# M4THYOU/TokenDagger

Measured on AMD Instinct MI355X. Metric: GB/s raw text tokenized (Llama-4 vocab, 1024 MB corpus), higher is better.
Workload: dtype u8; 1 GPU; Llama-4-Scout vocab, 1024 MiB synthetic english text, 1741775 documents, CoreBPE::encode semantics, input resident in HBM; bytes=1073741824, docs=1741775, bytes_rank0=1073741824, docs_rank0=1741775, parallelism=single GPU

## Files before the change

tokendagger_amd/csrc/td_kernels.hip:

```cpp
#include <hip/hip_runtime.h>
#include <stdlib.h>

#include "td_kernels.h"

namespace td {

#ifdef TD_ABLATE
#define TD_STOP(n) (a.stop_after == (n))
#else
#define TD_STOP(n) false
#endif

struct LdsSrc {
    const uint8_t* txt;
    const uint32_t* docw;
    int64_t lo, hi;
    __device__ __forceinline__ uint32_t byte(int64_t i) const { return txt[i]; }
    __device__ __forceinline__ bool doc(int64_t i) const { return (docw[i >> 5] >> (i & 31)) & 1u; }
};
struct GlobSrc {
    const uint8_t* text;
    const uint32_t* docbits;
    int64_t lo, hi;
    __device__ __forceinline__ uint32_t byte(int64_t i) const { return text[i]; }
// ... 3858 lines not shown
        bool fast_this = false;
        uint4 sx0 = cx0, sx1 = cx0, sx2 = cx0, sx3 = cx0;
        uint32_t sh0 = 0, stl = 0, sdsl = 0;
        int64_t sdpos = 0;
        if (SKIP_PLAIN && lane_walk) {
            bool done = false;
            while (!lw_cur) {
                if (!lw_nz) {
                    lw_base += nwaves * 64;
                    if (lw_base >= n_mwords) { done = true; break; }
                    lw_mine = lw_base + lane < n_mwords ? (walk_all ? 0xFFFFu : (uint32_t)a.rest_mask[lw_base + lane]) : 0u;
                    lw_nz = __ballot(lw_mine != 0u);
                    if (!lw_nz) continue;
                }
                const int l = td_ctz64(lw_nz);
                lw_nz &= lw_nz - 1ull;
                lw_cur = (uint32_t)__shfl((int)lw_mine, l);
                lw_index = lw_base + l;
            }
            if (done) break;
            const int bq = (int)td_ctz32(lw_cur);
            lw_cur &= lw_cur - 1u;
            tile = lw_index * 16 + bq;
            if (tile >= a.n_tiles) continue;
            tc = a.tile_count[tile]; ex = a.tile_extra[tile]; dfirst = (int64_t)a.tile_first_doc[tile];
            base = a.tile_base[tile] + a.chunk_pref[tile / K_SCAN_CHUNK];
            if (pk_simple(tc, base, ex, a.out_cap) || (a.pack_dense && pk_dense(tc, base, ex, a.out_cap))) continue;
        } else if constexpr (SKIP_PLAIN) {
            if (!cmask) {
                t0 += 4 * nwaves;
                if (t0 >= a.n_tiles) break;
                uint32_t w[4] = {0, 0, 0, 0};
#pragma unroll
                for (int q = 0; q < 4; ++q) {
                    const int tq = t0 + q * nwaves;
                    if (tq < a.n_tiles) w[q] = walk_all ? 0xFFFFu : (uint32_t)a.rest_mask[tq >> 4];
                }
#pragma unroll
                for (int q = 0; q < 4; ++q) {
                    const int tq = t0 + q * nwaves;
                    if (tq < a.n_tiles && ((w[q] >> (tq & 15)) & 1u)) cmask |= 1u << q;
                }
#pragma unroll
                for (int q = 0; q < 4; ++q) {
                    const int tq = t0 + q * nwaves;
                    if ((cmask >> q) & 1u) {
                        c_tc[q] = a.tile_count[tq]; c_ex[q] = a.tile_extra[tq]; c_df[q] = a.tile_first_doc[tq];
                        c_base[q] = a.tile_base[tq] + a.chunk_pref[tq / K_SCAN_CHUNK];
                    }
                }
                if (!cmask) continue;
            }
            const int q = (int)td_ctz32(cmask);
            cmask &= cmask - 1u;
            tile = t0 + q * nwaves;
            tc = q == 0 ? c_tc[0] : q == 1 ? c_tc[1] : q == 2 ? c_tc[2] : c_tc[3];
            ex = q == 0 ? c_ex[0] : q == 1 ? c_ex[1] : q == 2 ? c_ex[2] : c_ex[3];
            dfirst = (int64_t)(q == 0 ? c_df[0] : q == 1 ? c_df[1] : q == 2 ? c_df[2] : c_df[3]);
            base = q == 0 ? c_base[0] : q == 1 ? c_base[1] : q == 2 ? c_base[2] : c_base[3];
            if (pk_simple(tc, base, ex, a.out_cap) || (a.pack_dense && pk_dense(tc, base, ex, a.out_cap))) continue;
        } else {
            tile += nwaves;
            if (tile >= a.n_tiles) break;
            if (tile + 2 * nwaves < a.n_tiles) PK_FETCH(tile + 2 * nwaves, C)
            const bool fast_next = tile + nwaves < a.n_tiles && PK_FAST(B);
            if (fast_next) PK_LOAD(tile + nwaves, B, n)
            tc = tcA;
            base = baseA;
            dfirst = (int64_t)dfA;
            fast_this = fast_cur;
            sx0 = cx0; sx1 = cx1; sx2 = cx2; sx3 = cx3;
            sh0 = ch0; stl = ctl; sdsl = cdsl;
            sdpos = cdpos;
            tcA = tcB; baseA = baseB; dfA = dfB; tcB = tcC; baseB = baseC; dfB = dfC;
            fast_cur = fast_next;
            cx0 = nx0; cx1 = nx1; cx2 = nx2; cx3 = nx3; ch0 = nh0; ctl = ntl; cdsl = ndsl; cdpos = ndpos;
        }
        (void)ex;
        if (PLAIN_ONLY && !fast_this) continue;
        if (tc & TILE_DIRECT) {
            if (tile == a.n_tiles - 1) {
                const int64_t d_end = lower_bound_i64(a.doc_offsets, a.n_docs, a.n);
                for (int64_t d = d_end + lane; d <= a.n_docs; d += 64) a.out_offsets[d] = total;
            }
            continue;
        }
        if (fast_this && !TD_STOP(61)) {
            const uint32_t g_c = tc & TILE_COUNT_MASK;
            int32_t* dst = a.out_tokens + base;
            uint32_t g_head = (uint32_t)((16u - ((uint32_t)(uintptr_t)dst & 15u)) & 15u) >> 2;
            if (g_head > g_c) g_head = g_c;
            const uint32_t g_nv = (g_c - g_head) >> 2, g_done = g_head + 4 * g_nv;
            if ((uint32_t)lane < g_nv) *reinterpret_cast<uint4*>(dst + g_head + 4 * lane) = sx0;
            if ((uint32_t)lane + 64 < g_nv) *reinterpret_cast<uint4*>(dst + g_head + 4 * (lane + 64)) = sx1;
            if ((uint32_t)lane + 128 < g_nv) *reinterpret_cast<uint4*>(dst + g_head + 4 * (lane + 128)) = sx2;
            if ((uint32_t)lane + 192 < g_nv) *reinterpret_cast<uint4*>(dst + g_head + 4 * (lane + 192)) = sx3;
            if ((uint32_t)lane < g_head) dst[lane] = (int32_t)sh0;
            if (g_done + (uint32_t)lane < g_c) dst[g_done + lane] = (int32_t)stl;
            const int64_t g_lo = (int64_t)tile * K_TILE;
            const int64_t g_hi = (g_lo + K_TILE < a.n) ? g_lo + K_TILE : a.n;
            const int64_t dm = dfirst + lane;
            if (sdpos < g_hi) a.out_offsets[dm] = base + sdsl;
            if (__all(sdpos < g_hi)) {
                for (int64_t d = dfirst + 64 + lane; d < a.n_docs; d += 64) {
                    if (a.doc_offsets[d] >= g_hi) break;
                    a.out_offsets[d] = base + a.doc_slot[d];
                }
            }
            if (tile == a.n_tiles - 1) {
                const int64_t d_end = lower_bound_i64(a.doc_offsets, a.n_docs, a.n);
                for (int64_t d = d_end + lane; d <= a.n_docs; d += 64) a.out_offsets[d] = total;
            }
            continue;
        }
        if constexpr (PLAIN_ONLY) continue;
        const uint32_t cnt = tc & TILE_COUNT_MASK;
        const uint32_t* src = a.stage + (size_t)tile * K_STAGE;
        const int64_t g_lo = (int64_t)tile * K_TILE;
        const int64_t g_hi = (g_lo + K_TILE < a.n) ? g_lo + K_TILE : a.n;
        PK_TICK(t_meta)
        if (!(tc & (TILE_HAS_LONG | TILE_HAS_MISS | TILE_MISS_LISTED)) || TD_STOP(60)) {
            const int64_t dm = dfirst + lane;
            int64_t dpos = a.n;
            uint32_t dsl = 0;
            if (dm < a.n_docs) { dpos = a.doc_offsets[dm]; dsl = a.doc_slot[dm]; }
            if (base + cnt <= a.out_cap) {
                int32_t* dst = a.out_tokens + base;
                uint32_t head = (uint32_t)((16u - ((uint32_t)(uintptr_t)dst & 15u)) & 15u) >> 2;
                if (head > cnt) head = cnt;
                const uint32_t nv = (cnt - head) >> 2;
                const uint32_t done = head + 4 * nv;
                uint32_t h0 = 0, tl = 0;
                if ((uint32_t)lane < head) h0 = src[lane];
                if (done + (uint32_t)lane < cnt) tl = src[done + lane];
                for (uint32_t v0 = 0; v0 < nv; v0 += 256) {
                    uint4 x[4];
#pragma unroll
                    for (int q = 0; q < 4; ++q) {
                        const uint32_t v = v0 + q * 64 + lane;
                        if (v < nv) __builtin_memcpy(&x[q], src + head + 4 * v, 16);
                    }
#pragma unroll
                    for (int q = 0; q < 4; ++q) {
                        const uint32_t v = v0 + q * 64 + lane;
                        if (v < nv) *reinterpret_cast<uint4*>(dst + head + 4 * v) = x[q];
                    }
                }
                if ((uint32_t)lane < head) dst[lane] = (int32_t)h0;
                if (done + (uint32_t)lane < cnt) dst[done + lane] = (int32_t)tl;
            }
            if (dpos < g_hi) a.out_offsets[dm] = base + dsl;
            if (__all(dpos < g_hi)) {
                for (int64_t d = dfirst + 64 + lane; d < a.n_docs; d += 64) {
                    if (a.doc_offsets[d] >= g_hi) break;
                    a.out_offsets[d] = base + a.doc_slot[d];
                }
            }
        } else {
            unsigned long long* const elist = s_elist[wv];
            uint32_t ecount = 0;
            const uint64_t lt = (1ull << lane) - 1ull;
            auto flush = [&]() {
                PK_TICK(t_list)
                wave_sync();
                for (uint32_t c0 = 0; c0 < ecount; c0 += 64) {
                    const unsigned long long e = c0 + lane < ecount ? elist[c0 + lane] : 0ull;
                    const uint32_t n = (uint32_t)e & 127u;
                    const uint32_t* ps = marker_ids(a, (uint32_t)tile, (uint32_t)e);
                    const int64_t o = base + (int64_t)(uint32_t)(e >> 32);
                    for (uint32_t j = 0; __any(j < n); j += 4) {
                        uint32_t t[4];
#pragma unroll
                        for (uint32_t q = 0; q < 4; ++q) t[q] = j + q < n ? ps[j + q] : 0u;
#pragma unroll
                        for (uint32_t q = 0; q < 4; ++q)
                            if (j + q < n && o + j + q < a.out_cap) a.out_tokens[o + j + q] = (int32_t)t[q];
                    }
                }
                ecount = 0;
                wave_sync();
                PK_TICK(t_flush)
            };
            int64_t dnext = dfirst, dmine = 0;
            uint32_t dslot = 0xFFFFFFFFu;
            bool dfull = false;
            auto load_docs = [&]() {
                dmine = dnext + lane;
                const bool ok = dmine < a.n_docs && a.doc_offsets[dmine] < g_hi;
                dslot = ok ? a.doc_slot[dmine] : 0xFFFFFFFFu;
                dfull = __all(ok);
                dnext += 64;
            };
            load_docs();
            uint32_t carry = 0;
            for (uint32_t r0 = 0; r0 * 64u < cnt; r0 += PK_G) {
                uint32_t v[PK_G], sz[PK_G], off[PK_G];
                uint32_t lmask = 0, mmask = 0;
#pragma unroll
                for (int q = 0; q < PK_G; ++q) {
                    const uint32_t k = (r0 + q) * 64u + lane;
                    v[q] = k < cnt ? src[k] : 0u;
                }
#pragma unroll
                for (int q = 0; q < PK_G; ++q) {
                    const uint32_t k = (r0 + q) * 64u + lane;
                    const bool is_long = k < cnt && (v[q] & TOK_LONGREF) != 0, is_miss = k < cnt && !is_long && (v[q] & TOK_MISS);
                    lmask |= (is_long ? 1u : 0u) << q;
                    mmask |= (is_miss ? 1u : 0u) << q;
                    sz[q] = k < cnt ? (is_miss ? (v[q] & 127u) : 1u) : 0u;
                }
                PK_TICK(t_rows)
                const bool anylong = __any(lmask != 0);
                if (anylong) {
#pragma unroll
                    for (int q = 0; q < PK_G; ++q)
                        if ((lmask >> q) & 1u) sz[q] = a.long_list[v[q] & 0x7FFFFFFFu].ntok;
                }
#pragma unroll
                for (int q = 0; q < PK_G; ++q) {
                    const uint32_t r = r0 + q, k = r * 64u + lane;
                    const uint32_t incl = __any(((lmask | mmask) >> q) & 1u) ? wave_incl_scan(sz[q], lane)
                                        : ((r * 64u < cnt && cnt - r * 64u < 64u && k >= cnt) ? cnt - r * 64u : (r * 64u < cnt ? (uint32_t)lane + 1u : 0u));
                    off[q] = carry + incl - sz[q];
                    carry += (uint32_t)__builtin_amdgcn_readlane((int)incl, 63);
                }
                PK_TICK(t_scan)
#pragma unroll
                for (int q = 0; q < PK_G; ++q) {
                    const uint32_t k = (r0 + q) * 64u + lane;
                    const int64_t o = base + off[q];
                    if (k < cnt && !(((lmask | mmask) >> q) & 1u) && o < a.out_cap) a.out_tokens[o] = (int32_t)v[q];
                }
                PK_TICK(t_plain)
#pragma unroll
                for (int q = 0; q < PK_G; ++q) {
                    const bool m = (mmask >> q) & 1u;
                    const uint64_t bm = __ballot(m);
                    if (bm) {
                        if (m) elist[ecount + (uint32_t)__popcll((unsigned long long)(bm & lt))] = ((unsigned long long)off[q] << 32) | (v[q] & 0x1FFFFFFFu);
                        ecount += (uint32_t)__popcll((unsigned long long)bm);
                        if (ecount > (uint32_t)PK_ECAP - 64u) flush();
                    }
                }
                if (anylong) {
#pragma unroll
                    for (int q = 0; q < PK_G; ++q) {
                        for (uint64_t lb = __ballot((lmask >> q) & 1u); lb; lb &= lb - 1ull) {
                            const int l = (int)td_ctz64(lb);
                            const LongEntry le = a.long_list[(uint32_t)__shfl((int)v[q], l) & 0x7FFFFFFFu];
                            const int64_t lo = base + (int64_t)(uint32_t)__shfl((int)off[q], l);
                            const uint32_t* ps = a.pool + le.pool_off;
                            for (uint32_t j = lane; j < le.ntok; j += 64)
                                if (lo + j < a.out_cap) a.out_tokens[lo + j] = (int32_t)ps[j];
                        }
                    }
                }
                PK_TICK(t_list)
                for (;;) {
                    uint32_t pref = 0;
#pragma unroll
                    for (int q = 0; q < PK_G; ++q) {
                        const uint32_t pq = (uint32_t)__shfl((int)off[q], (int)(dslot & 63u));
                        if ((dslot >> 6) == r0 + (uint32_t)q) pref = pq;
                    }
                    if (dslot != 0xFFFFFFFFu && (dslot >> 6) >= r0 && (dslot >> 6) < r0 + (uint32_t)PK_G) a.out_offsets[dmine] = base + pref;
                    const uint32_t last = (uint32_t)__shfl((int)dslot, 63);
                    if (dfull && (last >> 6) < r0 + (uint32_t)PK_G) { load_docs(); continue; }
                    break;
                }
                PK_TICK(t_docs)
            }
            flush();
#ifdef TD_PACK_TIMING
            ++n_mt;
#endif
        }
#ifdef TD_PACK_TIMING
        if (!(tc & (TILE_HAS_LONG | TILE_HAS_MISS | TILE_MISS_LISTED))) { PK_TICK(t_plainpath) ++n_pt; }
#endif
        if (tile == a.n_tiles - 1) {
            const int64_t d_end = lower_bound_i64(a.doc_offsets, a.n_docs, a.n);
            for (int64_t d = d_end + lane; d <= a.n_docs; d += 64) a.out_offsets[d] = total;
        }
    }
#ifdef TD_PACK_TIMING
    if (lane == 0 && (blockIdx.x % 257) == 0 && wv == 0)
        printf("pack wave b%d: total %llu meta %llu plainpath %llu (%llu tiles) | marker tiles %llu: rows %llu scan %llu plain %llu list %llu flush %llu docs %llu\n", (int)blockIdx.x,
               (unsigned long long)(__builtin_readcyclecounter() - t_total0), t_meta, t_plainpath, n_pt, n_mt, t_rows, t_scan, t_plain, t_list, t_flush, t_docs);
#endif
}
__global__ __launch_bounds__(K_THREADS, 4) void td_pack_tokens(const EncodeArgs a) {
    __shared__ unsigned long long s_elist[K_THREADS / 64][PK_ECAP];
    pack_body<false, false>(a, s_elist);
}
#ifndef TD_PACK_PLAIN_WAVES
#define TD_PACK_PLAIN_WAVES 6
#endif
__global__ __launch_bounds__(K_THREADS, TD_PACK_PLAIN_WAVES) void td_pack_plain(const EncodeArgs a) {
    const int lane = threadIdx.x & 63;
    const int nwaves = gridDim.x * (K_THREADS / 64);
    for (int tile = blockIdx.x * (K_THREADS / 64) + (threadIdx.x >> 6); tile < a.n_tiles; tile += nwaves) {
        const uint32_t tc = a.tile_count[tile], ex = a.tile_extra[tile];
        const int64_t tb = a.tile_base[tile], cp = a.chunk_pref[tile / K_SCAN_CHUNK];
        const int64_t dfirst = (int64_t)a.tile_first_doc[tile];
        const uint32_t cnt = tc & TILE_COUNT_MASK;
        const int64_t base = tb + cp;
        if (!pk_simple(tc, base, ex, a.out_cap)) continue;
        const uint32_t* src = a.stage + (size_t)tile * K_STAGE;
        int32_t* dst = a.out_tokens + base;
        uint32_t v[16];
#pragma unroll
        for (int q = 0; q < 16; ++q) {
            const uint32_t k = (uint32_t)lane + 64u * q;
            v[q] = k < cnt ? src[k] : 0u;
        }
        const int64_t g_lo = (int64_t)tile * K_TILE;
        const int64_t g_hi = (g_lo + K_TILE < a.n) ? g_lo + K_TILE : a.n;
        const bool marks = (tc & TILE_MISS_LISTED) != 0;
        if (!marks) {
            for (int64_t d = dfirst + lane; d < a.n_docs; d += 64) {
                if (a.doc_offsets[d] >= g_hi) break;
                a.out_offsets[d] = base + a.doc_slot[d];
            }
#pragma unroll
            for (int q = 0; q < 16; ++q) {
                const uint32_t k = (uint32_t)lane + 64u * q;
                if (k < cnt) dst[k] = (int32_t)v[q];
            }
        } else {
            uint32_t sh[16], carry = 0;
#pragma unroll
            for (int q = 0; q < 16; ++q) {
                const bool m = (v[q] & 0xC0000000u) == TOK_MISS;
                uint32_t excl = 0, rowsum = 0;
                if (__ballot(m)) {
                    const uint32_t dlt = m ? (v[q] & 127u) - 1u : 0u;
                    const uint32_t incl = wave_incl_scan(dlt, lane);
                    excl = incl - dlt;
                    rowsum = (uint32_t)__builtin_amdgcn_readlane((int)incl, 63);
                }
                sh[q] = carry + excl;
                carry += rowsum;
            }
            for (int64_t d = dfirst + lane; __any(d < a.n_docs); d += 64) {
                const bool mine = d < a.n_docs && a.doc_offsets[d < a.n_docs ? d : 0] < g_hi;
                if (!__any(mine)) break;
                const uint32_t ks = mine ? a.doc_slot[d] : 0u;
                uint32_t s0 = 0;
#pragma unroll
                for (int q = 0; q < 16; ++q) {
                    const uint32_t t = (uint32_t)__shfl((int)sh[q], (int)(ks & 63u));
                    if ((ks >> 6) == (uint32_t)q) s0 = t;
                }
                if (mine) a.out_offsets[d] = base + (int64_t)(int32_t)(ks + (ks < cnt ? s0 : carry));
                if (!__all(mine)) break;
            }
#pragma unroll
            for (int q = 0; q < 16; ++q) {
                const uint32_t k = (uint32_t)lane + 64u * q;
                if (k < cnt) {
                    int32_t* o = dst + (int64_t)(int32_t)(k + sh[q]);
                    if ((v[q] & 0xC0000000u) == TOK_MISS) {
                        const uint32_t* mo = marker_ids(a, (uint32_t)tile, v[q]);
                        const uint32_t nt = v[q] & 127u;
                        for (uint32_t i = 0; i < nt; ++i) o[i] = (int32_t)mo[i];
                    } else {
                        *o = (int32_t)v[q];
                    }
                }
            }
        }
        if (tile == a.n_tiles - 1) {
            const int64_t total = a.tile_base[a.n_tiles];
            const int64_t d_end = lower_bound_i64(a.doc_offsets, a.n_docs, a.n);
            for (int64_t d = d_end + lane; d <= a.n_docs; d += 64) a.out_offsets[d] = total;
        }
    }
}
template <bool MULTI>
__device__ __forceinline__ void pack_dense_tile(const EncodeArgs& a, unsigned long long* const elist, const int tile, const uint32_t cnt, const int64_t base,
                                                const int64_t dfirst, const int lane) {
    const uint32_t* src = a.stage + (size_t)tile * K_STAGE;
    const int64_t g_lo = (int64_t)tile * K_TILE;
    const int64_t g_hi = (g_lo + K_TILE < a.n) ? g_lo + K_TILE : a.n;
    uint32_t ecount = 0;
    const uint64_t lt = (1ull << lane) - 1ull;
    auto flush = [&]() {
        wave_sync();
        for (uint32_t c0 = 0; c0 < ecount; c0 += 64) {
            const unsigned long long e = c0 + lane < ecount ? elist[c0 + lane] : 0ull;
            const uint32_t n = (uint32_t)e & 127u;
            const uint32_t* ps = marker_ids(a, (uint32_t)tile, (uint32_t)e);
            const int64_t o = base + (int64_t)(uint32_t)(e >> 32);
            for (uint32_t j = 0; __any(j < n); j += 4) {
                uint32_t t[4];
#pragma unroll
                for (uint32_t u = 0; u < 4; ++u) t[u] = j + u < n ? ps[j + u] : 0u;
#pragma unroll
                for (uint32_t u = 0; u < 4; ++u)
                    if (j + u < n) a.out_tokens[o + j + u] = (int32_t)t[u];
            }
        }
        ecount = 0;
        wave_sync();
    };
    uint32_t carry = 0;
    for (uint32_t s0 = 0;; s0 += 1024u) {
        uint32_t v[16];
#pragma unroll
        for (int q = 0; q < 16; ++q) {
            const uint32_t k = s0 + (uint32_t)lane + 64u * q;
            v[q] = k < cnt ? src[k] : 0u;
        }
        int64_t dm = dfirst + lane;
        bool dmine = dm < a.n_docs && a.doc_offsets[dm < a.n_docs ? dm : 0] < g_hi;
        uint32_t dks = dmine ? a.doc_slot[dm] : 0u;
        uint32_t lmask = 0, mmask = 0;
        uint32_t off[16];
#pragma unroll
        for (int q = 0; q < 16; ++q) {
            const uint32_t k = s0 + (uint32_t)lane + 64u * q;
            const bool is_long = k < cnt && (v[q] & TOK_LONGREF) != 0u, is_miss = k < cnt && !is_long && (v[q] & TOK_MISS) != 0u;
            lmask |= (is_long ? 1u : 0u) << q;
            mmask |= (is_miss ? 1u : 0u) << q;
            off[q] = k < cnt ? (is_miss ? (v[q] & 127u) : 1u) : 0u;
        }
        const bool anylong = __any(lmask != 0u);
        if (anylong) {
#pragma unroll
            for (int q = 0; q < 16; ++q)
                if ((lmask >> q) & 1u) off[q] = a.long_list[v[q] & 0x7FFFFFFFu].ntok;
        }
#pragma unroll
        for (int q = 0; q < 16; ++q) {
            const uint32_t r64 = s0 + 64u * (uint32_t)q, k = r64 + (uint32_t)lane;
            const uint32_t sz = off[q];
            const uint32_t incl = __any(((lmask | mmask) >> q) & 1u) ? wave_incl_scan(sz, lane)
                                : ((r64 < cnt && cnt - r64 < 64u && k >= cnt) ? cnt - r64 : (r64 < cnt ? (uint32_t)lane + 1u : 0u));
            off[q] = carry + incl - sz;
            carry += (uint32_t)__builtin_amdgcn_readlane((int)incl, 63);
        }
        const bool last_seg = !MULTI || s0 + 1024u >= cnt;
        for (;;) {
            const uint32_t rel = dks - s0;
            uint32_t pref = carry;
#pragma unroll
            for (int q = 0; q < 16; ++q) {
                const uint32_t t = (uint32_t)__shfl((int)off[q], (int)(rel & 63u));
                if ((rel >> 6) == (uint32_t)q) pref = t;
            }
            const bool in_seg = dmine && dks < cnt && dks >= s0 && rel < 1024u, behind = dmine && dks >= cnt && last_seg;
            if (in_seg || behind) a.out_offsets[dm] = base + (int64_t)(behind ? carry : pref);
            if (!__all(dmine)) break;
            dm += 64;
            dmine = dm < a.n_docs && a.doc_offsets[dm < a.n_docs ? dm : 0] < g_hi;
            dks = dmine ? a.doc_slot[dm] : 0u;
            if (!__any(dmine)) break;
        }
#pragma unroll
        for (int q = 0; q < 16; ++q) {
            const uint32_t k = s0 + (uint32_t)lane + 64u * q;
            if (k < cnt && !(((lmask | mmask) >> q) & 1u)) a.out_tokens[base + off[q]] = (int32_t)v[q];
        }
        if (__any(mmask != 0u)) {
#pragma unroll
            for (int q = 0; q < 16; ++q) {
                const bool m = (mmask >> q) & 1u;
                const uint64_t bm = __ballot(m);
                if (bm) {
                    if (m) elist[ecount + (uint32_t)__popcll((unsigned long long)(bm & lt))] = ((unsigned long long)off[q] << 32) | (v[q] & 0x1FFFFFFFu);
                    ecount += (uint32_t)__popcll((unsigned long long)bm);
                    if (ecount > (uint32_t)PK_ECAP - 64u) flush();
                }
            }
        }
        if (anylong) {
#pragma unroll
            for (int q = 0; q < 16; ++q) {
                for (uint64_t lb = __ballot((lmask >> q) & 1u); lb; lb &= lb - 1ull) {
                    const int l = (int)td_ctz64(lb);
                    const LongEntry le = a.long_list[(uint32_t)__shfl((int)v[q], l) & 0x7FFFFFFFu];
                    const int64_t lo = base + (int64_t)(uint32_t)__shfl((int)off[q], l);
                    const uint32_t* ps = a.pool + le.pool_off;
                    for (uint32_t j = lane; j < le.ntok; j += 64) a.out_tokens[lo + j] = (int32_t)ps[j];
                }
            }
        }
        if (last_seg) break;
    }
    if (ecount) flush();
    if (tile == a.n_tiles - 1) {
        const int64_t total = a.tile_base[a.n_tiles];
        const int64_t d_end = lower_bound_i64(a.doc_offsets, a.n_docs, a.n);
        for (int64_t d = d_end + lane; d <= a.n_docs; d += 64) a.out_offsets[d] = total;
    }
}
#ifndef TD_PACK_DENSE_WAVES
#define TD_PACK_DENSE_WAVES 5
#endif
template <bool MULTI>
__global__ __launch_bounds__(K_THREADS, MULTI ? 4 : TD_PACK_DENSE_WAVES) void td_pack_dense(const EncodeArgs a) {
    __shared__ unsigned long long s_elist[K_THREADS / 64][PK_ECAP];
    const int lane = threadIdx.x & 63, wv = threadIdx.x >> 6;
    const int tile = blockIdx.x * (K_THREADS / 64) + wv;
    if (tile >= a.n_tiles) return;
    const uint32_t tc = a.tile_count[tile], ex = a.tile_extra[tile];
    const int64_t tb = a.tile_base[tile], cp = a.chunk_pref[tile / K_SCAN_CHUNK];
    const int64_t dfirst = (int64_t)a.tile_first_doc[tile];
    const uint32_t cnt = tc & TILE_COUNT_MASK;
    const int64_t base = tb + cp;
    if (!pk_dense(tc, base, ex, a.out_cap)) return;
    if ((cnt > 1024u) != MULTI) return;
    pack_dense_tile<MULTI>(a, s_elist[wv], tile, cnt, base, dfirst, lane);
}
__global__ __launch_bounds__(K_THREADS) void td_pack_rest(const EncodeArgs a) {
    __shared__ unsigned long long s_elist[K_THREADS / 64][PK_ECAP];
    pack_body<false, true>(a, s_elist);
}

constexpr int SM_MAXBYTES = K_TILE;
constexpr int SM_LONG_MAX = 64;
struct SmallCfAcc {
    using pos_t = int;
    const uint8_t* cfs;
    const uint8_t* txt;
    int lim;
    __device__ __forceinline__ uint32_t cf(int i) const { return cfs[i]; }
    __device__ __forceinline__ uint32_t byte(int i) const { return txt[i]; }
};
__device__ __forceinline__ void small_encode_body(const SmallArgs& a) {
    __shared__ __attribute__((aligned(16))) uint8_t s_txt[SM_MAXBYTES + 80];
    __shared__ __attribute__((aligned(16))) uint8_t s_cf[SM_MAXBYTES + 80];
    __shared__ uint32_t s_doc[SM_MAXBYTES / 32 + 4];
    __shared__ uint32_t s_start[SM_MAXBYTES / 32 + 4];
    __shared__ uint16_t s_plist[SM_MAXBYTES + 8];
    __shared__ __attribute__((aligned(16))) uint32_t s_tok[SM_MAXBYTES + 64];
    __shared__ __attribute__((aligned(16))) uint32_t s_keys[K_THREADS * MG_UNIT];
    __shared__ __attribute__((aligned(16))) uint32_t s_ids[K_THREADS * MG_UNIT];
    __shared__ uint16_t s_miss[SM_MAXBYTES / 2 + 8];
    __shared__ uint32_t s_off[K_THREADS];
    __shared__ uint16_t s_valid[K_THREADS];
    __shared__ int32_t s_byteid[256];
    __shared__ uint32_t s_wave[8];
    __shared__ uint32_t s_nmiss, s_err, s_errpos, s_fallback;
    __shared__ uint32_t s_nlong;
    __shared__ uint16_t s_long[SM_LONG_MAX];
    __shared__ uint16_t s_doff[SM_MAXDOCS + 2];

    const int tid = threadIdx.x;
    const Tables T = uniform_tables(a.Tp);
    const int n = a.n;
    for (int d = tid; d <= a.n_docs && d <= SM_MAXDOCS; d += K_THREADS) {
        const int64_t p = a.doc_offsets[d];
        s_doff[d] = (uint16_t)(p < 0 ? n : p > n ? n : p);
    }
    for (int q = tid; q < 256; q += K_THREADS) s_byteid[q] = T.byte_id[q];
    for (int q = tid; q < (SM_MAXBYTES + 80) / 16; q += K_THREADS) {
        uint4 v = make_uint4(0, 0, 0, 0);
        if (q * 16 + 16 <= n) v = reinterpret_cast<const uint4*>(a.text)[q];
        else if (q * 16 < n)
            for (int k = 0; k < 16 && q * 16 + k < n; ++k) reinterpret_cast<uint8_t*>(&v)[k] = a.text[q * 16 + k];
        reinterpret_cast<uint4*>(s_txt)[q] = v;
    }
    for (int q = tid; q < SM_MAXBYTES / 32 + 4; q += K_THREADS) { s_doc[q] = 0; s_start[q] = 0; }
    for (int q = tid; q < (SM_MAXBYTES + 64) / 4; q += K_THREADS) reinterpret_cast<uint4*>(s_tok)[q] = make_uint4(TOK_NONE, TOK_NONE, TOK_NONE, TOK_NONE);
    if (tid == 0) { s_nmiss = 0; s_err = 0; s_errpos = 0; s_fallback = 0; s_nlong = 0; }
    __syncthreads();
    for (int d = tid; d < a.n_docs; d += K_THREADS) {
        const int p = s_doff[d];
        if (p < n) atomicOr(&s_doc[p >> 5], 1u << (p & 31));
    }
    __syncthreads();
    auto fail = [&](int code, int pos) { if (atomicCAS(&s_err, 0u, (uint32_t)code) == 0u) s_errpos = (uint32_t)pos; };
    {
        LdsSrc src;
        src.txt = s_txt; src.docw = s_doc; src.lo = 0; src.hi = n;
        for (int i = tid; i < SM_MAXBYTES + 80; i += K_THREADS) {
            uint32_t v = F_DOC;
            if (i < n) {
                v = classify_at(T, src, i);
                if (src.doc(i)) v |= F_DOC;
            }
            s_cf[i] = (uint8_t)v;
        }
    }
    __syncthreads();
    {
        const SmallCfAcc A{s_cf, s_txt, n + 64};
        const int c0 = tid * K_CHUNK, c1 = c0 + K_CHUNK;
        int s = -1;
        if (c0 < n) {
            const int cend = c1 < n ? c1 : n;
            for (int i = c0; i < cend; ++i)
                if (is_sync(i > 0 ? s_cf[i - 1] : 0u, s_cf[i], T.pat_flags)) { s = i; break; }
        }
        for (int p = s; p >= 0 && p < n;) {
            if (p >= c1 && is_sync(s_cf[p - 1], s_cf[p], T.pat_flags)) break;
            atomicOr(&s_start[p >> 5], 1u << (p & 31));
            p = scan_piece(A, p, T.pat_flags);
        }
    }
    __syncthreads();
    uint32_t np_total;
    {
        const int c0 = tid * K_CHUNK;
        uint32_t smask = (c0 < n) ? (s_start[c0 >> 5] >> (c0 & 31)) & 0xFFFFu : 0u;
        if (c0 + K_CHUNK > n && c0 < n) smask &= (1u << (n - c0)) - 1u;
        const uint32_t pbase = block_excl_scan(__popc(smask), s_wave, np_total);
        uint32_t k = pbase;
        while (smask) {
            const int b = __ffs(smask) - 1;
            smask &= smask - 1;
            s_plist[k++] = (uint16_t)(c0 + b);
        }
        if (tid == 0) s_plist[np_total] = (uint16_t)n;
    }
    __syncthreads();
    for (uint32_t k = tid; k < np_total; k += K_THREADS) {
        const int i = s_plist[k];
        const uint32_t len = (uint32_t)s_plist[k + 1] - (uint32_t)i;
        const uint8_t* pb = s_txt + i;
        if (len == 1) {
            const int32_t id = s_byteid[pb[0]];
            if (id >= T.pseudo_base) fail(TD_E_UNKNOWN_BYTE, i);
            s_tok[i] = (uint32_t)id;
            continue;
        }
        if (len > (uint32_t)K_MAXSHORT) {
            uint32_t at = (uint32_t)SM_LONG_MAX;
            if (len <= (uint32_t)LP_MEDIUM) at = atomicAdd(&s_nlong, 1u);
            if (at < (uint32_t)SM_LONG_MAX) s_long[at] = (uint16_t)k; else s_fallback = 1;
            continue;
        }
        int32_t r = NO_RANK;
        if (a.use_fastpath) {
            auto get = [pb](uint32_t q) { return (uint32_t)pb[q]; };
            uint64_t key = 0;
            if (len <= 8) for (uint32_t q = 0; q < len; ++q) key |= (uint64_t)pb[q] << (8 * q);
            else key = hash_bytes(get, len);
            r = piece_lookup(T, key, len, get);
        }
        if (r != NO_RANK) s_tok[i] = (uint32_t)r;
        else s_miss[atomicAdd(&s_nmiss, 1u)] = (uint16_t)k;
    }
    __syncthreads();
    {
        const uint32_t nmiss = s_nmiss;
        for (int pass = 0; pass < 2; ++pass) {
            const uint32_t u = pass == 0 ? 1u : 4u;
            const uint32_t per = (uint32_t)K_THREADS / u;
            uint32_t done = 0;
            while (done < nmiss) {
                MergeState st;
                st.alive = 0; st.t = (uint32_t)tid; st.len = 0;
                int pos = 0;
                uint32_t taken = 0, scan = done;
                while (scan < nmiss && taken < per) {
                    const uint32_t k = s_miss[scan];
                    const uint32_t len = (uint32_t)s_plist[k + 1] - (uint32_t)s_plist[k];
                    if ((len <= 16u) == (pass == 0)) {
                        if ((uint32_t)tid == taken * u) { st.len = len; pos = s_plist[k]; }
                        ++taken;
                    }
                    ++scan;
                }
                done = scan;
                if (st.len) {
                    st.alive = st.len >= 64u ? ~0ull : ((1ull << st.len) - 1ull);
                    for (uint32_t j = 0; j < st.len; ++j) mg_put(T, s_byteid, s_keys, s_ids, st, j, s_txt[pos + j], s_txt[pos + j + 1]);
                    mg_pad(s_keys, st);
                }
                for (;;) {
                    const bool more = mg_round_t<uint64_t>(T, s_keys, s_ids, st);
                    if (!__any(more)) break;
                }
                if (st.len) {
                    for (uint64_t al = st.alive; al; al &= al - 1ull) {
                        const uint32_t j = (uint32_t)td_ctz64(al);
// ... 610 lines not shown
```

Measured before the change: 465.8 GB/s.

## Restructure pack_plain marker path into single pass with wave-parallel marker expansion

Hoists the first per-lane document offset/slot load ahead of the token staging loads so its latency overlaps them. In the marker tile path, it merges the shift scan, document-offset lookup and plain-token stores into one pass over the rows. It collects up to 64 marker entries into lanes and expands them cooperatively across the wave instead of one serial loop per lane. Markers beyond 64 and extra document batches fall back to a rescan of the stage buffer, which costs more on dense tiles, and compiler barriers (empty asm) pin values to scalar or vector registers.

Result: no change. 469.0 GB/s, median of 6 (+0.7%).

```diff
diff --git a/tokendagger_amd/csrc/td_kernels.hip b/tokendagger_amd/csrc/td_kernels.hip
--- a/tokendagger_amd/csrc/td_kernels.hip
+++ b/tokendagger_amd/csrc/td_kernels.hip
@@ -4184,12 +4184,17 @@
     for (int tile = blockIdx.x * (K_THREADS / 64) + (threadIdx.x >> 6); tile < a.n_tiles; tile += nwaves) {
         const uint32_t tc = a.tile_count[tile], ex = a.tile_extra[tile];
         const int64_t tb = a.tile_base[tile], cp = a.chunk_pref[tile / K_SCAN_CHUNK];
-        const int64_t dfirst = (int64_t)a.tile_first_doc[tile];
+        uint32_t df = a.tile_first_doc[tile];
+        asm volatile("" : "+v"(df));
+        const int64_t dfirst = (int64_t)df;
         const uint32_t cnt = tc & TILE_COUNT_MASK;
         const int64_t base = tb + cp;
         if (!pk_simple(tc, base, ex, a.out_cap)) continue;
         const uint32_t* src = a.stage + (size_t)tile * K_STAGE;
         int32_t* dst = a.out_tokens + base;
+        const int64_t dm = dfirst + lane, dc = dm < a.n_docs ? dm : 0;
+        const int64_t dpos = a.doc_offsets[dc];
+        const uint32_t dks = a.doc_slot[dc];
         uint32_t v[16];
 #pragma unroll
         for (int q = 0; q < 16; ++q) {
@@ -4198,11 +4203,20 @@
         }
         const int64_t g_lo = (int64_t)tile * K_TILE;
         const int64_t g_hi = (g_lo + K_TILE < a.n) ? g_lo + K_TILE : a.n;
+        const bool dmine = dm < a.n_docs && dpos < g_hi;
         const bool marks = (tc & TILE_MISS_LISTED) != 0;
+#ifdef TD_PACK_TIMING
+        if (lane == 0 && (tile & 63) == 0) printf("pack_plain tile %d marks %d\n", tile, (int)marks);
+#endif
         if (!marks) {
-            for (int64_t d = dfirst + lane; d < a.n_docs; d += 64) {
-                if (a.doc_offsets[d] >= g_hi) break;
-                a.out_offsets[d] = base + a.doc_slot[d];
+            if (dmine) {
+                a.out_offsets[dm] = base + dks;
+                uint32_t more = 64;
+                asm volatile("" : "+s"(more));
+                for (int64_t d = dm + more; d < a.n_docs; d += 64) {
+                    if (a.doc_offsets[d] >= g_hi) break;
+                    a.out_offsets[d] = base + a.doc_slot[d];
+                }
             }
 #pragma unroll
             for (int q = 0; q < 16; ++q) {
@@ -4210,52 +4224,100 @@
                 if (k < cnt) dst[k] = (int32_t)v[q];
             }
         } else {
-            uint32_t sh[16], carry = 0;
-#pragma unroll
-            for (int q = 0; q < 16; ++q) {
-                const bool m = (v[q] & 0xC0000000u) == TOK_MISS;
-                uint32_t excl = 0, rowsum = 0;
-                if (__ballot(m)) {
-                    const uint32_t dlt = m ? (v[q] & 127u) - 1u : 0u;
-                    const uint32_t incl = wave_incl_scan(dlt, lane);
-                    excl = incl - dlt;
-                    rowsum = (uint32_t)__builtin_amdgcn_readlane((int)incl, 63);
-                }
-                sh[q] = carry + excl;
-                carry += rowsum;
-            }
-            for (int64_t d = dfirst + lane; __any(d < a.n_docs); d += 64) {
-                const bool mine = d < a.n_docs && a.doc_offsets[d < a.n_docs ? d : 0] < g_hi;
-                if (!__any(mine)) break;
-                const uint32_t ks = mine ? a.doc_slot[d] : 0u;
-                uint32_t s0 = 0;
-#pragma unroll
-                for (int q = 0; q < 16; ++q) {
-                    const uint32_t t = (uint32_t)__shfl((int)sh[q], (int)(ks & 63u));
-                    if ((ks >> 6) == (uint32_t)q) s0 = t;
-                }
-                if (mine) a.out_offsets[d] = base + (int64_t)(int32_t)(ks + (ks < cnt ? s0 : carry));
-                if (!__all(mine)) break;
-            }
+            auto row_scan = [&](uint32_t vq, uint32_t& rowsum) {
+                const uint32_t dlt = (vq & 0xC0000000u) == TOK_MISS ? (vq & 127u) - 1u : 0u;
+                const uint32_t incl = wave_incl_scan(dlt, lane);
+                rowsum = (uint32_t)__builtin_amdgcn_readlane((int)incl, 63);
+                return incl - dlt;
+            };
+            uint32_t carry = 0;
+            uint32_t dsh = 0;
+            uint32_t nm = 0;
+            uint32_t lv = 0, lo = 0;
 #pragma unroll
             for (int q = 0; q < 16; ++q) {
                 const uint32_t k = (uint32_t)lane + 64u * q;
-                if (k < cnt) {
-                    int32_t* o = dst + (int64_t)(int32_t)(k + sh[q]);
-                    if ((v[q] & 0xC0000000u) == TOK_MISS) {
-                        const uint32_t* mo = marker_ids(a, (uint32_t)tile, v[q]);
-                        const uint32_t nt = v[q] & 127u;
-                        for (uint32_t i = 0; i < nt; ++i) o[i] = (int32_t)mo[i];
-                    } else {
-                        *o = (int32_t)v[q];
+                const bool m = (v[q] & 0xC0000000u) == TOK_MISS;
+                const uint64_t bm = __ballot(m);
+                uint32_t shift = carry;
+                if (bm) {
+                    uint32_t rowsum;
+                    shift += row_scan(v[q], rowsum);
+                    const uint32_t t = (uint32_t)__shfl((int)shift, (int)(dks & 63u));
+                    if ((dks >> 6) == (uint32_t)q) dsh = t;
+                    for (uint64_t b = bm; b; b &= b - 1ull, ++nm) {
+                        const int l = (int)td_ctz64(b);
+                        const uint32_t pv = (uint32_t)__builtin_amdgcn_readlane((int)v[q], l), po = (uint32_t)__builtin_amdgcn_readlane((int)(k + shift), l);
+                        if ((uint32_t)lane == nm) { lv = pv; lo = po; }
                     }
+                    carry += rowsum;
+                } else if ((dks >> 6) == (uint32_t)q) {
+                    dsh = carry;
+                }
+                if (k < cnt && !m) dst[(int64_t)(int32_t)(k + shift)] = (int32_t)v[q];
+            }
+            if (dmine) a.out_offsets[dm] = base + (int64_t)(int32_t)(dks + (dks < cnt ? dsh : carry));
+            {
+                const uint32_t nl = nm < 64u ? nm : 64u;
+                const uint32_t* mp = marker_ids(a, (uint32_t)tile, (uint32_t)lane < nl ? lv : 0u);
+                for (uint32_t j = 0; j < nl; ++j) {
+                    const uint32_t nt = (uint32_t)__builtin_amdgcn_readlane((int)lv, (int)j) & 127u;
+                    const uint64_t pj = (uint64_t)(uintptr_t)mp;
+                    const uint32_t* ps = (const uint32_t*)(uintptr_t)(((uint64_t)(uint32_t)__builtin_amdgcn_readlane((int)(uint32_t)(pj >> 32), (int)j) << 32) |
+                                                                    (uint32_t)__builtin_amdgcn_readlane((int)(uint32_t)pj, (int)j));
+                    int32_t* o = dst + (int64_t)(int32_t)__builtin_amdgcn_readlane((int)lo, (int)j);
+                    for (uint32_t i = lane; i < nt; i += 64u) o[i] = (int32_t)ps[i];
+                }
+            }
+            if (nm > 64u) {
+                const uint64_t lt = (1ull << lane) - 1ull;
+                uint32_t c2 = 0, seen = 0;
+#pragma unroll 1
+                for (uint32_t k = lane; k < cnt + (uint32_t)lane; k += 64u) {
+                    const uint32_t vq = k < cnt ? src[k] : 0u;
+                    const bool m = (vq & 0xC0000000u) == TOK_MISS;
+                    const uint64_t bm = __ballot(m);
+                    if (!bm) continue;
+                    uint32_t rowsum;
+                    const uint32_t shift = c2 + row_scan(vq, rowsum);
+                    if (m && seen + (uint32_t)__popcll((unsigned long long)(bm & lt)) >= 64u) {
+                        const uint32_t* ps = marker_ids(a, (uint32_t)tile, vq);
+                        int32_t* o = dst + (int64_t)(int32_t)(k + shift);
+                        for (uint32_t i = 0; i < (vq & 127u); ++i) o[i] = (int32_t)ps[i];
+                    }
+                    seen += (uint32_t)__popcll((unsigned long long)bm);
+                    c2 += rowsum;
+                }
+            }
+            if (__all(dmine)) {
+                uint32_t more = 64;
+                asm volatile("" : "+s"(more));
+                for (int64_t d = dm + more;; d += 64) {
+                    const bool mine = d < a.n_docs && a.doc_offsets[d < a.n_docs ? d : 0] < g_hi;
+                    if (!__any(mine)) break;
+                    const uint32_t ks = mine ? a.doc_slot[d] : 0u;
+                    uint32_t c2 = 0, s0 = 0;
+#pragma unroll 1
+                    for (uint32_t r = 0; r * 64u < cnt; ++r) {
+                        const uint32_t k = r * 64u + (uint32_t)lane;
+                        const uint32_t vq = k < cnt ? src[k] : 0u;
+                        uint32_t shift = c2, rowsum = 0;
+                        if (__ballot((vq & 0xC0000000u) == TOK_MISS)) shift += row_scan(vq, rowsum);
+                        const uint32_t t = (uint32_t)__shfl((int)shift, (int)(ks & 63u));
+                        if ((ks >> 6) == r) s0 = t;
+                        c2 += rowsum;
+                    }
+                    if (mine) a.out_offsets[d] = base + (int64_t)(int32_t)(ks + (ks < cnt ? s0 : carry));
+                    if (!__all(mine)) break;
                 }
             }
         }
         if (tile == a.n_tiles - 1) {
-            const int64_t total = a.tile_base[a.n_tiles];
-            const int64_t d_end = lower_bound_i64(a.doc_offsets, a.n_docs, a.n);
-            for (int64_t d = d_end + lane; d <= a.n_docs; d += 64) a.out_offsets[d] = total;
+            const int64_t total = a.tile_base[tile + 1];
+            int64_t nd = a.n_docs;
+            asm volatile("" : "+s"(nd));
+            const int64_t d_end = lower_bound_i64(a.doc_offsets, nd, a.n);
+            for (int64_t d = d_end + lane; d <= nd; d += 64) a.out_offsets[d] = total;
         }
     }
 }
```
